# zzuiekongning/MGDT-YOLO

Measured on AMD Instinct MI355X. Metric: images/sec @640x640 bs=32 per GPU, detection forward + NMS (whole job: 1 GPU(s)), higher is better.
Workload: dtype bf16; 1 GPU; mspa_c2f_gd_yolov8-n (MSPA-C2f + GD neck + Detect, nc=80) 640x640 inference, batch 32/GPU: forward + decode + NMS(conf 0.25, iou 0.7), hipGraph replay, 4 batches in flight (one captured graph per resident batch, replayed round-robin on 4 streams); global_batch=32, parallelism=replicas x1 (batch-sharded, no data-path collective), rccl_ranks=1, input=bfloat16 NCHW images, 8 different batches resident in HBM (600 MiB) cycled, detections_last_step=9600, weights=seeded random init (no checkpoints offline), batches_in_flight=4

## Files before the change

### mgdt_yolo_amd/csrc/csp_block.hip

```cpp
#include <algorithm>
#include <vector>

#include "conv_igemm_kernel.h"

struct CspArgs {
  const char* x; int xsn, xsh, xsw; uint32_t x_bytes;
  char* y; int ysn, ysh, ysw; uint32_t y_bytes;
  const char* front; const float* front_bias;
  const char* mid[4]; const float* mid_bias[4];
  const char* back; const float* back_bias;
  float* pool;
  int N, H, W, Cin, Cout, wd, nbtl, shortcut, act;
  int TH, TW, halo, RH, RW, tiles_x, tiles_y, total_tiles, per_xcd;
  int catC, nchb, nbo;
  int RPA, TPA, CS;
  int catS, cmsk, csh;
  int chain_words;
  unsigned long long* dbg;
  int pool_gst;
  FastDiv fd_rw, fd_tw, fd_tx, fd_tpi;
};

constexpr int CSP_THREADS = 512;
constexpr int CSP_NW = CSP_THREADS / 64;
constexpr int CSP_NCHB_MAX = 8;

__device__ __forceinline__ float csp_act(float v, int) { return v * fast_sigmoid(v); }

typedef __attribute__((__vector_size__(2 * sizeof(unsigned int)))) unsigned int csp_raw2;

__device__ __forceinline__ void lds_store4(char* p, f32x4 v) {
  bf16x4 o;
#pragma unroll
  for (int i = 0; i < 4; ++i) o[i] = (bf16)v[i];
  *(bf16x4*)p = o;
}
template <int WD> __device__ __forceinline__ int csp_psw(int pix) { return WD == 64 ? (pix & 7) : (WD == 32 ? ((pix >> 1) & 3) : 0); }

__device__ __forceinline__ f32x4 lds_load4(const char* p) {
  const bf16x4 o = *(const bf16x4*)p;
  return f32x4{(float)o[0], (float)o[1], (float)o[2], (float)o[3]};
}

__device__ __forceinline__ csp_raw2 csp_swap32(unsigned int lo, unsigned int hi) { return __builtin_amdgcn_permlane32_swap(lo, hi, false, false); }
__device__ __forceinline__ f32x4 csp_merge(f32x4 va, f32x4 vb) {
  f32x4 m;
#pragma unroll
  for (int j = 0; j < 4; ++j) {
    const float fa = va[j], fb = vb[j];
    m[j] = __uint_as_float(csp_swap32(__float_as_uint(fa), __float_as_uint(fb))[0]);
  }
  return m;
}

template <int WD, int MODE, bool PAIR = false>
__global__ __launch_bounds__(CSP_THREADS, (WD <= 32 ? 4 : 2)) void csp_block_kernel(const CspArgs a) {
  static_assert(!PAIR || (WD == 8 && MODE == 0), "the paired epilogue is the wd = 8 MSPA form");
  constexpr int CP = WD / 8;
  constexpr int NCHB = WD == 8 ? 2 : (WD == 16 ? 3 : (WD == 32 ? 5 : 8));
  constexpr int NB = WD >= 16 ? WD / 16 : 1;
  constexpr int NCH = (9 * CP + 3) / 4;
  constexpr int NBK = NB, KC = (NBK + 1) / 2;
  constexpr int PS = 2 * WD;
  extern __shared__ __attribute__((aligned(16))) char smem[];
  char* Pb = smem;
  char* Tb = Pb + (size_t)a.RPA * PS;
  char* catb = Tb + (size_t)a.RPA * PS;
  char* wl = catb + (size_t)a.TPA * a.CS;

  const int tid = threadIdx.x, lane = tid & 63;
  const int wave = __builtin_amdgcn_readfirstlane(tid >> 6);
  const int r = lane & 15, g = lane >> 4;

  const int v = blockIdx.x;
  const int tlin = (v & 7) * a.per_xcd + (v >> 3);
  if ((v >> 3) >= a.per_xcd || tlin >= a.total_tiles) return;
  const int tpi = a.tiles_x * a.tiles_y;
  const int n = (int)fdiv((uint32_t)tlin, a.fd_tpi), trem = tlin - n * tpi;
  const int tyi = (int)fdiv((uint32_t)trem, a.fd_tx);
  const int ty0 = tyi * a.TH, tx0 = (trem - tyi * a.tiles_x) * a.TW;
  const int RP = a.RH * a.RW, TP = a.TH * a.TW;
  const bool inner = ty0 >= a.halo && tx0 >= a.halo && ty0 + a.TH + a.halo <= a.H && tx0 + a.TW + a.halo <= a.W;
  auto stamp = [&](int k) __attribute__((always_inline)) { if (a.dbg && tid == 0) a.dbg[(size_t)tlin * 8 + k] = __builtin_amdgcn_s_memrealtime(); };
  auto region_px = [&](int q, int& go, int& ct) __attribute__((always_inline)) {
    const int ry = (int)fdiv((uint32_t)q, a.fd_rw), rx = q - ry * a.RW;
    const int iy = ty0 - a.halo + ry, ix = tx0 - a.halo + rx;
    go = (q < RP && (unsigned)iy < (unsigned)a.H && (unsigned)ix < (unsigned)a.W) ? n * a.xsn + iy * a.xsh + ix * a.xsw : MGDT_OOB;
    const int cy = ry - a.halo, cx = rx - a.halo;
    ct = (q < RP && (unsigned)cy < (unsigned)a.TH && (unsigned)cx < (unsigned)a.TW) ? cy * a.TW + cx : -1;
  };
  auto pt_at = [&](int q, int c) __attribute__((always_inline)) { return q * PS + ((((c >> 3) ^ csp_psw<WD>(q)) << 4) | ((c & 7) << 1)); };
  auto cat_at = [&](int t, int c) __attribute__((always_inline)) { return t * a.CS + ((((c >> 3) ^ ((t >> a.csh) & a.cmsk)) << 4) | ((c & 7) << 1)); };
  stamp(0);

  const int nbv = wave % NB, gvm = wave / NB, gstm = CSP_NW / NB;
  bf16x8 A[NCH];
  f32x4 bias;
  auto load_a0 = [&]() __attribute__((always_inline)) {
#pragma unroll
    for (int kc = 0; kc < NCH; ++kc) A[kc] = *(const bf16x8*)(a.mid[0] + ((size_t)(kc * NB + nbv) * 64 + lane) * 16);
    bias = *(const f32x4*)(a.mid_bias[0] + nbv * 16 + 4 * g);
  };
  if (WD != 32 || MODE != 0) load_a0();

  {
    const int words = (int)(((size_t)2 * a.RPA * PS) >> 4);
    uint4* z = (uint4*)Pb;
    for (int i = tid; i < words; i += CSP_THREADS) z[i] = make_uint4(0u, 0u, 0u, 0u);
  }
  if (MODE == 0) {
    for (int i = tid; i < a.chain_words; i += CSP_THREADS) ((uint4*)wl)[i] = ((const uint4*)a.front)[i];
    float* bl = (float*)(wl + (size_t)a.chain_words * 16);
    for (int i = tid; i < 3 * NBK * 16; i += CSP_THREADS) bl[i] = ((const float*)(a.front + (size_t)a.chain_words * 16))[i];
  }
  __syncthreads();
  stamp(1);

  const __amdgpu_buffer_rsrc_t xrs = __builtin_amdgcn_make_buffer_rsrc((void*)a.x, 0, a.x_bytes, 0x00020000);
  const __amdgpu_buffer_rsrc_t yrs = __builtin_amdgcn_make_buffer_rsrc((void*)a.y, 0, a.y_bytes, 0x00020000);
  const int ngr = (RP + 15) >> 4;

  if (MODE == 0) {
    constexpr int U = WD == 64 ? 2 : (WD == 32 ? 3 : 5);
    const char* const wlane = wl + lane * 16;
    const float* bl = (const float*)(wl + (size_t)a.chain_words * 16);
    const int per = ngr / CSP_NW, rem = ngr - per * CSP_NW;
    const int gbeg = wave * per + min(wave, rem), gend = gbeg + per + (wave < rem ? 1 : 0);
    if constexpr (PAIR) {
      constexpr int UP = 3;
      const int hb = lane >> 5, cl = 4 * (g & 1);
      for (int g0 = gbeg; g0 < gend; g0 += 2 * UP) {
        int go[UP], ct[UP];
        csp_raw2 XR[UP][4];
#pragma unroll
        for (int u = 0; u < UP; ++u) {
          const int grp = g0 + 2 * u + hb;
          region_px(grp * 16 + r, go[u], ct[u]);
          if (grp >= gend) go[u] = MGDT_OOB, ct[u] = -1;
#pragma unroll
          for (int i = 0; i < 4; ++i) XR[u][i] = __builtin_amdgcn_raw_buffer_load_b64(xrs, (uint32_t)go[u] + (uint32_t)((i * WD + cl) * 2), 0, 0);
        }
#pragma unroll
        for (int u = 0; u < UP; ++u) {
          if (g0 + 2 * u >= gend) break;
          const bool hasb = g0 + 2 * u + 1 < gend;
          const int q = (g0 + 2 * u + hb) * 16 + r;
          f32x4 X[4];
#pragma unroll
          for (int i = 0; i < 4; ++i) {
            const bf16x4 o = __builtin_bit_cast(bf16x4, XR[u][i]);
            X[i] = f32x4{(float)o[0], (float)o[1], (float)o[2], (float)o[3]};
          }
          f32x4 prev;
#pragma unroll
          for (int i = 0; i < 3; ++i) {
            bf16x4 vb;
#pragma unroll
            for (int e = 0; e < 4; ++e) vb[e] = (bf16)(X[i][e] + (i ? prev[e] : 0.f));
            const csp_raw2 vw = __builtin_bit_cast(csp_raw2, vb);
            const csp_raw2 s0 = csp_swap32(vw[0], 0u), s1 = csp_swap32(vw[1], 0u);
            typedef __attribute__((__vector_size__(4 * sizeof(unsigned int)))) unsigned int raw4;
            const bf16x8 Ba = __builtin_bit_cast(bf16x8, (raw4){s0[0], s1[0], 0u, 0u});
            const bf16x8 Bb = __builtin_bit_cast(bf16x8, (raw4){s0[1], s1[1], 0u, 0u});
            const f32x4 bi = *(const f32x4*)(bl + i * 16 + 4 * g);
            const bf16x8 Wf = *(const bf16x8*)(wlane + i * 1024);
            const f32x4 acca = mma(Wf, Ba, bi);
            f32x4 accb = bi;
            if (hasb) accb = mma(Wf, Bb, bi);
            f32x4 acc = csp_merge(acca, accb);
#pragma unroll
            for (int j = 0; j < 4; ++j) acc[j] = (float)(bf16)csp_act(acc[j], a.act);
            prev = acc;
            if (ct[u] >= 0) lds_store4(catb + cat_at(ct[u], i * WD + cl), acc);
          }
          f32x4 p0 = prev + X[3];
          if (go[u] == MGDT_OOB) p0 = f32x4{0.f, 0.f, 0.f, 0.f};
          if (hb == 0 || hasb) lds_store4(Pb + pt_at(q, cl), p0);
        }
      }
    } else
    for (int g0 = gbeg; g0 < gend; g0 += U) {
      int go[U], ct[U];
      csp_raw2 XR[U][4][NBK];
#pragma unroll
      for (int u = 0; u < U; ++u) {
        const bool gv_ = g0 + u < gend;
        const int q = (g0 + u) * 16 + r;
        region_px(q, go[u], ct[u]);
        if (!gv_) go[u] = MGDT_OOB, ct[u] = -1;
#pragma unroll
        for (int i = 0; i < 4; ++i)
#pragma unroll
          for (int blk = 0; blk < NBK; ++blk) {
            const int c = blk * 16 + 4 * g;
            const int dead = c >= WD ? MGDT_OOB : 0;
            XR[u][i][blk] = __builtin_amdgcn_raw_buffer_load_b64(xrs, (uint32_t)(go[u] | dead) + (uint32_t)((i * WD + c) * 2), 0, 0);
          }
      }
#pragma unroll
      for (int u = 0; u < U; ++u) {
        if (g0 + u >= gend) break;
        const int q = (g0 + u) * 16 + r;
        f32x4 X[4][NBK];
#pragma unroll
        for (int i = 0; i < 4; ++i)
#pragma unroll
          for (int blk = 0; blk < NBK; ++blk) {
            const bf16x4 o = __builtin_bit_cast(bf16x4, XR[u][i][blk]);
            X[i][blk] = f32x4{(float)o[0], (float)o[1], (float)o[2], (float)o[3]};
          }
        f32x4 prev[NBK];
#pragma unroll
        for (int i = 0; i < 3; ++i) {
          bf16x8 Bf[KC];
#pragma unroll
          for (int kc = 0; kc < KC; ++kc)
#pragma unroll
            for (int e = 0; e < 8; ++e) {
              const int blk = kc * 2 + e / 4;
              float vv = 0.f;
              if (blk < NBK) vv = X[i][blk][e % 4] + (i ? prev[blk][e % 4] : 0.f);
              Bf[kc][e] = (bf16)vv;
            }
#pragma unroll
          for (int ob = 0; ob < NBK; ++ob) {
            f32x4 acc = *(const f32x4*)(bl + (i * NBK + ob) * 16 + 4 * g);
#pragma unroll
            for (int kc = 0; kc < KC; ++kc) acc = mma(*(const bf16x8*)(wlane + ((i * KC + kc) * NBK + ob) * 1024), Bf[kc], acc);
#pragma unroll
            for (int j = 0; j < 4; ++j) acc[j] = (float)(bf16)csp_act(acc[j], a.act);
            prev[ob] = acc;
            const int c = ob * 16 + 4 * g;
            if (c < WD && ct[u] >= 0) lds_store4(catb + cat_at(ct[u], i * WD + c), acc);
          }
        }
#pragma unroll
        for (int ob = 0; ob < NBK; ++ob) {
          const int c = ob * 16 + 4 * g;
          f32x4 p0 = prev[ob] + X[3][ob];
          if (go[u] == MGDT_OOB) p0 = f32x4{0.f, 0.f, 0.f, 0.f};
          if (c < WD) lds_store4(Pb + pt_at(q, c), p0);
        }
      }
    }
  } else {
    constexpr int NB2 = 2 * WD / 16;
    constexpr int U = WD == 64 ? 2 : 4;
    const int per = ngr / CSP_NW, rem = ngr - per * CSP_NW;
    const int gbeg = wave * per + min(wave, rem), gend = gbeg + per + (wave < rem ? 1 : 0);
    for (int g0 = gbeg; g0 < gend; g0 += U) {
      int go[U], ct[U];
      csp_raw2 XR[U][NB2];
#pragma unroll
      for (int u = 0; u < U; ++u) {
        const bool gv_ = g0 + u < gend;
        const int q = (g0 + u) * 16 + r;
        region_px(q, go[u], ct[u]);
        if (!gv_) go[u] = MGDT_OOB, ct[u] = -1;
#pragma unroll
        for (int blk = 0; blk < NB2; ++blk)
          XR[u][blk] = __builtin_amdgcn_raw_buffer_load_b64(xrs, (uint32_t)go[u] + (uint32_t)((blk * 16 + 4 * g) * 2), 0, 0);
      }
#pragma unroll
      for (int u = 0; u < U; ++u) {
        if (g0 + u >= gend) break;
        const int q = (g0 + u) * 16 + r;
#pragma unroll
        for (int blk = 0; blk < NB2; ++blk) {
          const int cc = blk * 16 + 4 * g;
          if (ct[u] >= 0) *(csp_raw2*)(catb + cat_at(ct[u], cc)) = XR[u][blk];
          if (cc >= WD) *(csp_raw2*)(Pb + pt_at(q, cc - WD)) = XR[u][blk];
        }
      }
    }
  }
  if (WD == 32 && MODE == 0) load_a0();
  stamp(2);
  __syncthreads();
  stamp(3);

  constexpr bool PREB = WD <= 16;
  bf16x8 AB[NCHB];
  f32x4 biasB = f32x4{0.f, 0.f, 0.f, 0.f};
  const int bgst = a.pool_gst, bgv = wave / (CSP_NW / bgst), obst = CSP_NW / bgst, ob0 = wave % obst;
  {
    const int gv = gvm, gst = gstm;
    const int cch = nbv * 16 + 4 * g;
    const int slot0 = (MODE == 0 ? 3 : 2) * WD;
    for (int j = 0; j < 2 * a.nbtl; ++j) {
      const char* in = (j & 1) ? Tb : Pb;
      char* out = (j & 1) ? Pb : Tb;
      constexpr bool PREN = WD <= 16;
      bf16x8 An[PREN ? NCH : 1];
      f32x4 biasn = bias;
      const bool more = j + 1 < 2 * a.nbtl;
      if (more) {
        if (PREN) {
#pragma unroll
          for (int kc = 0; kc < NCH; ++kc) An[kc] = *(const bf16x8*)(a.mid[j + 1] + ((size_t)(kc * NB + nbv) * 64 + lane) * 16);
          biasn = *(const f32x4*)(a.mid_bias[j + 1] + nbv * 16 + 4 * g);
        }
      } else if (PREB && ob0 < a.nbo) {
#pragma unroll
        for (int kc = 0; kc < NCHB; ++kc)
          if (kc < a.nchb) AB[kc] = *(const bf16x8*)(a.back + ((size_t)(kc * a.nbo + ob0) * 64 + lane) * 16);
        biasB = *(const f32x4*)(a.back_bias + ob0 * 16 + 4 * g);
      }
      const int lo = (j + 1) * a.RW + (j + 1), hi = (a.RH - j - 2) * a.RW + (a.RW - j - 1);
      const int ng = (hi - lo + 15) >> 4;
      const bool second = j & 1;
      const bool tocat = second && (j >> 1) + 1 < a.nbtl;
      const bool zchk = !inner && j + 1 < 2 * a.nbtl;
      int boff[NCH];
#pragma unroll
      for (int kc = 0; kc < NCH; ++kc) {
        const int p = kc * 4 + g;
        int tap = p / CP, cp = p - tap * CP;
        if (tap >= 9) { tap = 4; cp = 0; }
        const int toff = (tap / 3 - 1) * a.RW + (tap % 3 - 1);
        boff[kc] = toff * PS + ((cp ^ csp_psw<WD>(lo + r + toff)) << 4);
      }
      auto finish = [&](int q, f32x4 acc, int cc, bool live) __attribute__((always_inline)) {
#pragma unroll
        for (int jj = 0; jj < 4; ++jj) acc[jj] = csp_act(acc[jj], a.act);
        if (live && q < hi && cc < WD) {
          char* po = out + pt_at(q, cc);
          if (second && a.shortcut) acc += lds_load4(po);
          int go = 0, ct = -1;
          if (zchk || tocat) region_px(q, go, ct);
          if (zchk && go == MGDT_OOB) acc = f32x4{0.f, 0.f, 0.f, 0.f};
          lds_store4(po, acc);
          if (tocat && ct >= 0) lds_store4(catb + cat_at(ct, slot0 + (j >> 1) * WD + cc), acc);
        }
      };
      for (int grp = gv; grp < ng; grp += 2 * gst) {
        const int qa = lo + grp * 16 + r;
        const bool hasb = grp + gst < ng;
        const int qb = hasb ? qa + gst * 16 : qa;
        const char* pa = in + qa * PS;
        const char* pb = in + qb * PS;
        f32x4 acca = bias, accb = bias;
#pragma unroll
        for (int kc = 0; kc < NCH; ++kc) {
          acca = mma(A[kc], *(const bf16x8*)(pa + boff[kc]), acca);
          accb = mma(A[kc], *(const bf16x8*)(pb + boff[kc]), accb);
        }
        if constexpr (PAIR) {
          finish(lane < 32 ? qa : qb, csp_merge(acca, accb), 4 * (g & 1), lane < 32 || hasb);
        } else {
          finish(qa, acca, cch, true);
          if (hasb) finish(qb, accb, cch, true);
        }
      }
      __syncthreads();
      if (j == 0) stamp(4);
      if (more) {
        if (PREN) {
#pragma unroll
          for (int kc = 0; kc < NCH; ++kc) A[kc] = An[kc];
          bias = biasn;
        } else {
#pragma unroll
          for (int kc = 0; kc < NCH; ++kc) A[kc] = *(const bf16x8*)(a.mid[j + 1] + ((size_t)(kc * NB + nbv) * 64 + lane) * 16);
          bias = *(const f32x4*)(a.mid_bias[j + 1] + nbv * 16 + 4 * g);
        }
      }
    }
  }
  stamp(5);

  {
    const int tg = (TP + 15) >> 4;
    const int nsl = a.catS >> 3, csw = (r >> a.csh) & a.cmsk;
    int koff[NCHB];
    bool kinp[NCHB];
#pragma unroll
    for (int kc = 0; kc < NCHB; ++kc) {
      const int p = kc * 4 + g;
      kinp[kc] = p >= nsl && p < nsl + CP;
      koff[kc] = kinp[kc] ? p - nsl : ((p < nsl ? p : 0) ^ csw) << 4;
    }
    const int gst = bgst, gv = bgv;
    bf16x8 ABn[PREB ? 1 : NCHB];
    f32x4 biasBn = biasB;
    if (!PREB && ob0 < a.nbo) {
#pragma unroll
      for (int kc = 0; kc < NCHB; ++kc)
        if (kc < a.nchb) AB[kc] = *(const bf16x8*)(a.back + ((size_t)(kc * a.nbo + ob0) * 64 + lane) * 16);
      biasB = *(const f32x4*)(a.back_bias + ob0 * 16 + 4 * g);
    }
    for (int ob = ob0; ob < a.nbo; ob += obst) {
      if (PREB && ob != ob0) {
#pragma unroll
        for (int kc = 0; kc < NCHB; ++kc)
          if (kc < a.nchb) AB[kc] = *(const bf16x8*)(a.back + ((size_t)(kc * a.nbo + ob) * 64 + lane) * 16);
        biasB = *(const f32x4*)(a.back_bias + ob * 16 + 4 * g);
      }
      if (!PREB && ob + obst < a.nbo) {
#pragma unroll
        for (int kc = 0; kc < NCHB; ++kc)
          if (kc < a.nchb) ABn[kc] = *(const bf16x8*)(a.back + ((size_t)(kc * a.nbo + ob + obst) * 64 + lane) * 16);
        biasBn = *(const f32x4*)(a.back_bias + (ob + obst) * 16 + 4 * g);
      }
      const int co = ob * 16 + 4 * g;
      const int dead = co >= a.Cout ? MGDT_OOB : 0;
      f32x4 psum = f32x4{0.f, 0.f, 0.f, 0.f};
      for (int grp = gv; grp < tg; grp += gst) {
        const int t = grp * 16 + r;
        const int tc = min(t, TP - 1);
        const int cy = (int)fdiv((uint32_t)tc, a.fd_tw), cx = tc - cy * a.TW;
        const int tq = (cy + a.halo) * a.RW + cx + a.halo;
        const int yo = t < TP ? n * a.ysn + (ty0 + cy) * a.ysh + (tx0 + cx) * a.ysw : MGDT_OOB;
        const char* pc = catb + t * a.CS;
        const char* pp = Pb + tq * PS;
        const int psw = csp_psw<WD>(tq);
        f32x4 acc = biasB;
#pragma unroll
        for (int kc = 0; kc < NCHB; ++kc)
          if (kc < a.nchb) acc = mma(AB[kc], *(const bf16x8*)(kinp[kc] ? pp + ((koff[kc] ^ psw) << 4) : pc + koff[kc]), acc);
#pragma unroll
        for (int jj = 0; jj < 4; ++jj) acc[jj] = (float)(bf16)csp_act(acc[jj], a.act);
        bstore4<bf16>(yrs, (uint32_t)(yo | dead) + (uint32_t)(co * 2), acc);
        if (t < TP) psum += acc;
      }
      if (a.pool) {
#pragma unroll
        for (int m = 1; m < 16; m <<= 1)
#pragma unroll
          for (int jj = 0; jj < 4; ++jj) psum[jj] += __shfl_xor(psum[jj], m, 64);
        if (r == 0 && co < a.Cout) {
          *(f32x4*)(a.pool + (((size_t)n * tpi + trem) * gst + gv) * a.Cout + co) = psum;
        }
      }
      if (!PREB && ob + obst < a.nbo) {
#pragma unroll
        for (int kc = 0; kc < NCHB; ++kc) AB[kc] = ABn[kc];
        biasB = biasBn;
      }
    }
  }
  stamp(6);
}

struct CspGeom { int TH, TW, halo, RH, RW, RPA, TPA, CS, tiles_x, tiles_y; size_t lds; };

static void csp_cat_swizzle(int slots, int* cmsk, int* csh) {
  if (slots % 16 == 0) { *cmsk = 15; *csh = 0; }
  else if (slots % 8 == 0) { *cmsk = 7; *csh = 0; }
  else if (slots % 4 == 0) { *cmsk = 3; *csh = 1; }
  else { *cmsk = 0; *csh = 0; }
}

static bool csp_geometry(int mode, int H, int W, int wd, int nbtl, int catC, size_t extra, int th, int tw, CspGeom* g) {
  g->TH = th; g->TW = tw; g->halo = 2 * nbtl;
  g->RH = th + 2 * g->halo; g->RW = tw + 2 * g->halo;
  const int RP = g->RH * g->RW;
  g->RPA = ((RP + 15 + 15) / 16) * 16;
  g->TPA = ((th * tw + 15) / 16) * 16;
  g->CS = (catC - wd) * 2;
  g->tiles_x = W / tw; g->tiles_y = H / th;
  g->lds = 2 * (size_t)g->RPA * (wd * 2) + (size_t)g->TPA * g->CS + extra;
  (void)mode;
  return g->lds <= 156 * 1024;
}

static int csp_chain_nbk(int wd) { return wd >= 16 ? wd / 16 : 1; }
static int csp_pool_gst(int cout) { const int nbo = (cout + 15) / 16; return (nbo < CSP_NW && CSP_NW % nbo == 0) ? CSP_NW / nbo : 1; }

int csp_c3_supported(int cin, int cout, int wd, int nbtl, int h, int w, int dtype);
int csp_c3_tiles(int n, int cin, int cout, int wd, int nbtl, int h, int w, int* geom8);
int csp_c3_fwd(const mgdt_view* x, const void* const* mid, const float* const* mid_bias, int nbtl, int shortcut, const void* back, const float* back_bias,
               int wd, const mgdt_view* y, mgdt_stream s);

extern "C" int mgdt_csp_block_supported(int mode, int cin, int cout, int wd, int nbtl, int h, int w, int dtype) {
  if (mode == 2) return csp_c3_supported(cin, cout, wd, nbtl, h, w, dtype);
  if (mode != 0 && mode != 1) return 0;
  if (dtype != MGDT_BF16 || (wd != 8 && wd != 16 && wd != 32 && wd != 64) || nbtl < 1 || nbtl > 2 || cout % 4) return 0;
  const int catC = (mode == 0 ? 3 : 2) * wd + nbtl * wd;
  if (catC > 256 || catC % 8) return 0;
  if (mode == 0) {
    if (cin != 4 * wd || h % 2 || w % 2 || h < 4 || w < 4) return 0;
  } else {
    if (cin != 2 * wd || wd < 16) return 0;
  }
  return 1;
}

constexpr size_t CSP_LDS_2WG = 80 * 1024;
constexpr double CSP_1WG_COST = 2.0;

static bool csp_pick_tile(int mode, int H, int W, int N, int wd, int nbtl, int catC, size_t extra, CspGeom* best) {
  const char* e = getenv("MGDT_CSP_TILE");
  int fth = 0, ftw = 0;
  if (e && sscanf(e, "%d,%d", &fth, &ftw) != 2) fth = ftw = 0;
  const int qh = mode == 0 ? H / 2 : H, qw = mode == 0 ? W / 2 : W;
  double best_cost = 1e30;
  bool found = false;
  for (int th = 2; th <= std::min(qh, 32); ++th) {
    if (qh % th) continue;
    for (int tw = 2; tw <= std::min(qw, 32); ++tw) {
      if (qw % tw) continue;
      if (fth && (th != fth || tw != ftw)) continue;
      CspGeom g;
      if (!csp_geometry(mode, H, W, wd, nbtl, catC, extra, th, tw, &g)) continue;
      const double wgs = (double)N * g.tiles_x * g.tiles_y;
      const double ratio = (double)(g.RH * g.RW) / (th * tw);
      const double fill = (double)(th * tw) / g.TPA;
      double cost = ratio / fill;
      if (wgs < 256) cost *= 256.0 / wgs;
      if (wd <= 32 && g.lds > CSP_LDS_2WG) cost *= CSP_1WG_COST;
      if (cost < best_cost) { best_cost = cost; *best = g; found = true; }
    }
  }
  return found;
}

extern "C" int mgdt_csp_block_tiles(int mode, int n, int cin, int cout, int wd, int nbtl, int h, int w, int* geom6) {
  if (mode == 2) return csp_c3_tiles(n, cin, cout, wd, nbtl, h, w, geom6);
  if (!mgdt_csp_block_supported(mode, cin, cout, wd, nbtl, h, w, MGDT_BF16)) return 0;
  const int catC = (mode == 0 ? 3 : 2) * wd + nbtl * wd;
  const int nbk = csp_chain_nbk(wd);
  const size_t extra = mode == 0 ? (size_t)3 * ((nbk + 1) / 2) * nbk * 1024 + 3 * nbk * 16 * 4 : 0;
  CspGeom g;
  if (!csp_pick_tile(mode, h, w, n, wd, nbtl, catC, extra, &g)) return 0;
  if (geom6) {
    geom6[0] = g.TH; geom6[1] = g.TW; geom6[2] = g.RH; geom6[3] = g.RW; geom6[4] = (int)g.lds; geom6[5] = n * g.tiles_x * g.tiles_y;
    geom6[6] = g.tiles_x; geom6[7] = g.tiles_y;
  }
  return g.tiles_x * g.tiles_y * csp_pool_gst(cout);
}

extern "C" int mgdt_csp_block_fwd(int mode, const mgdt_view* x, const void* front, const float* front_bias, const void* const* mid,
                                  const float* const* mid_bias, int nbtl, int shortcut, const void* back, const float* back_bias, int wd, int act,
                                  const mgdt_view* y, float* pool, int dtype, mgdt_stream s) {
  if (!view_ok(x) || !view_ok(y) || (mode == 0 && !front) || !mid || !mid_bias || !back || !back_bias) MGDT_FAIL(MGDT_BAD_ARG, "csp_block: null/empty argument");
  if (!mgdt_csp_block_supported(mode, x->c, y->c, wd, nbtl, x->h, x->w, dtype))
    MGDT_FAIL(MGDT_BAD_SHAPE, "csp_block: mode=%d cin=%d cout=%d wd=%d n=%d %dx%d dtype=%d not covered", mode, x->c, y->c, wd, nbtl, x->h, x->w, dtype);
  if (x->n != y->n || x->h != y->h || x->w != y->w) MGDT_FAIL(MGDT_BAD_SHAPE, "csp_block: x and y must have one spatial size");
  if (act != MGDT_ACT_SILU) MGDT_FAIL(MGDT_BAD_ARG, "csp_block: activation %d (only SiLU, the blocks' default, is built)", act);
  for (int j = 0; j < 2 * nbtl; ++j)
    if (!mid[j] || !mid_bias[j]) MGDT_FAIL(MGDT_BAD_ARG, "csp_block: missing conv panel %d", j);
  if (mode == 2) return csp_c3_fwd(x, mid, mid_bias, nbtl, shortcut, back, back_bias, wd, y, s);
  CspArgs a;
  memset(&a, 0, sizeof(a));
  const long sz = 2;
  bool fits = true;
  auto bind = [&](const mgdt_view* v, const char** p, int* sn, int* sh, int* sw, uint32_t* bytes, int q) {
    const long ext = ((long)(v->n - 1) * v->sn + (long)(v->h - 1) * v->sh + (long)(v->w - 1) * v->sw + v->c) * sz;
    if (v->sc != 1 || v->sw % q || v->sh % q || v->sn % q || (uintptr_t)v->p % (q * sz) || ext >= 0x7fffffffL) { fits = false; return; }
    *p = (const char*)v->p; *sn = (int)(v->sn * sz); *sh = (int)(v->sh * sz); *sw = (int)(v->sw * sz); *bytes = (uint32_t)ext;
  };
  const char* yp = nullptr;
  bind(x, &a.x, &a.xsn, &a.xsh, &a.xsw, &a.x_bytes, 4);
  bind(y, &yp, &a.ysn, &a.ysh, &a.ysw, &a.y_bytes, 4);
  if (!fits) MGDT_FAIL(MGDT_BAD_SHAPE, "csp_block: views must be aligned NHWC (sc == 1) and span < 2 GiB");
  a.y = (char*)yp;
  a.front = (const char*)front; a.front_bias = front_bias;
  for (int j = 0; j < 2 * nbtl; ++j) { a.mid[j] = (const char*)mid[j]; a.mid_bias[j] = mid_bias[j]; }
  a.back = (const char*)back; a.back_bias = back_bias; a.pool = pool;
  a.N = x->n; a.H = x->h; a.W = x->w; a.Cin = x->c; a.Cout = y->c; a.wd = wd; a.nbtl = nbtl; a.shortcut = shortcut; a.act = act;
  a.catC = (mode == 0 ? 3 : 2) * wd + nbtl * wd;
  a.nchb = (a.catC / 8 + 3) / 4; a.nbo = (a.Cout + 15) / 16; a.pool_gst = csp_pool_gst(a.Cout);
  const int nbk = csp_chain_nbk(wd);
  a.chain_words = mode == 0 ? 3 * ((nbk + 1) / 2) * nbk * 64 : 0;
  const size_t extra = mode == 0 ? (size_t)a.chain_words * 16 + 3 * nbk * 16 * 4 : 0;
  CspGeom g;
  if (!csp_pick_tile(mode, a.H, a.W, a.N, wd, nbtl, a.catC, extra, &g)) MGDT_FAIL(MGDT_BAD_SHAPE, "csp_block: no tile fits %dx%d wd=%d n=%d", a.H, a.W, wd, nbtl);
  a.TH = g.TH; a.TW = g.TW; a.halo = g.halo; a.RH = g.RH; a.RW = g.RW; a.tiles_x = g.tiles_x; a.tiles_y = g.tiles_y;
  a.RPA = g.RPA; a.TPA = g.TPA; a.CS = g.CS;
  a.catS = a.catC - wd;
  csp_cat_swizzle(a.catS / 8, &a.cmsk, &a.csh);
  a.total_tiles = a.N * g.tiles_x * g.tiles_y;
  a.fd_rw = make_fastdiv((uint32_t)g.RW); a.fd_tw = make_fastdiv((uint32_t)g.TW); a.fd_tx = make_fastdiv((uint32_t)g.tiles_x);
  a.fd_tpi = make_fastdiv((uint32_t)(g.tiles_x * g.tiles_y));
  a.per_xcd = cdiv(a.total_tiles, 8);
  const int grid = 8 * a.per_xcd;
  hipStream_t st = (hipStream_t)s;
  static unsigned long long* dbgbuf = nullptr;
  static size_t dbgcap = 0;
  if (getenv("MGDT_CSP_DBG") && dbgcap < (size_t)a.total_tiles * 8) {
    if (dbgbuf) (void)hipFree(dbgbuf);
    dbgcap = (size_t)a.total_tiles * 8;
    (void)hipMalloc((void**)&dbgbuf, dbgcap * 8);
  }
  a.dbg = getenv("MGDT_CSP_DBG") ? dbgbuf : nullptr;
  const char* ep = getenv("MGDT_CSP_PAIR");
  const bool pair = !(ep && ep[0] == '0');
#define CSP_LAUNCH(...)                                                                                              \
  do {                                                                                                                      \
    static std::atomic<bool> attr{false};                                                                                            \
    if (!attr) {                                                                                                            \
      hipError_t e_ = hipFuncSetAttribute((const void*)csp_block_kernel<__VA_ARGS__>, hipFuncAttributeMaxDynamicSharedMemorySize, 160 * 1024); \
      if (e_ != hipSuccess) MGDT_FAIL(MGDT_LAUNCH_FAIL, "csp_block: hipFuncSetAttribute: %s", hipGetErrorString(e_));         \
      attr = true;                                                                                                          \
    }                                                                                                                       \
    csp_block_kernel<__VA_ARGS__><<<grid, CSP_THREADS, g.lds, st>>>(a);                                                      \
  } while (0)
  if (mode == 0) {
    switch (wd) { case 8: if (pair) CSP_LAUNCH(8, 0, true); else CSP_LAUNCH(8, 0); break; case 16: CSP_LAUNCH(16, 0); break; case 32: CSP_LAUNCH(32, 0); break; default: CSP_LAUNCH(64, 0); break; }
  } else {
    switch (wd) { case 16: CSP_LAUNCH(16, 1); break; case 32: CSP_LAUNCH(32, 1); break; default: CSP_LAUNCH(64, 1); break; }
  }
#undef CSP_LAUNCH
  MGDT_CHECK_LAUNCH("csp_block_fwd");
  if (a.dbg) {
    std::vector<unsigned long long> h((size_t)a.total_tiles * 8);
    (void)hipStreamSynchronize(st);
    (void)hipMemcpy(h.data(), a.dbg, h.size() * 8, hipMemcpyDeviceToHost);
    unsigned long long t0 = ~0ull, t1 = 0;
    double ph[6] = {0, 0, 0, 0, 0, 0};
    for (int i = 0; i < a.total_tiles; ++i) {
      t0 = std::min(t0, h[(size_t)i * 8]); t1 = std::max(t1, h[(size_t)i * 8 + 6]);
      for (int k = 0; k < 6; ++k) ph[k] += (double)(h[(size_t)i * 8 + k + 1] - h[(size_t)i * 8 + k]);
    }
    const double nw = a.total_tiles;
    fprintf(stderr, "csp_block mode %d wd %d n %d %dx%d tile %dx%d (%d wgs, lds %zu): span %.1f us; avg per WG (us): tables %.2f front %.2f sync %.2f conv0 %.2f "
                    "other convs %.2f back %.2f\n", mode, wd, nbtl, a.H, a.W, g.TH, g.TW, a.total_tiles, g.lds, (t1 - t0) * 0.01, ph[0] / nw * 0.01,
            ph[1] / nw * 0.01, ph[2] / nw * 0.01, ph[3] / nw * 0.01, ph[4] / nw * 0.01, ph[5] / nw * 0.01);
  }
  return MGDT_OK;
}
```

Before: 40380 images/sec.

## Compact halo-shrinking conv walk and re-swizzle LDS reads in fused CSP block

The chained 3x3 convs in the fused CSP block now iterate only over the valid shrinking interior pixels. A fast division by the per-stage width maps a compact index back to region coordinates, so work is no longer wasted on row-wrap pixels between lo and hi. For wd>=32 the LDS read offsets use an XOR swizzle computed per pixel address, and weight and bias prefetch for the next stage or the back conv is moved before the barrier. The loop is split at compile time so the last stage is specialised, and occupancy for the paired wd=8 form rises to 6 waves per SIMD. The cost is extra integer work per pixel group and higher register pressure.

```diff
diff --git a/mgdt_yolo_amd/csrc/csp_block.hip b/mgdt_yolo_amd/csrc/csp_block.hip
--- a/mgdt_yolo_amd/csrc/csp_block.hip
+++ b/mgdt_yolo_amd/csrc/csp_block.hip
@@ -1,4 +1,5 @@
 #include <algorithm>
+#include <type_traits>
 #include <vector>
 
 #include "conv_igemm_kernel.h"
@@ -19,11 +20,13 @@
   unsigned long long* dbg;
   int pool_gst;
   FastDiv fd_rw, fd_tw, fd_tx, fd_tpi;
+  FastDiv fd_cw[4];
 };
 
 constexpr int CSP_THREADS = 512;
 constexpr int CSP_NW = CSP_THREADS / 64;
 constexpr int CSP_NCHB_MAX = 8;
+constexpr int csp_waves_per_simd(int wd, bool pair) { return wd == 8 && pair ? 6 : (wd <= 32 ? 4 : 2); }
 
 __device__ __forceinline__ float csp_act(float v, int) { return v * fast_sigmoid(v); }
 
@@ -53,8 +56,8 @@
   return m;
 }
 
-template <int WD, int MODE, bool PAIR = false>
-__global__ __launch_bounds__(CSP_THREADS, (WD <= 32 ? 4 : 2)) void csp_block_kernel(const CspArgs a) {
+template <int WD, int MODE, bool PAIR = false, bool COMPACT = true>
+__global__ __launch_bounds__(CSP_THREADS, csp_waves_per_simd(WD, PAIR)) void csp_block_kernel(const CspArgs a) {
   static_assert(!PAIR || (WD == 8 && MODE == 0), "the paired epilogue is the wd = 8 MSPA form");
   constexpr int CP = WD / 8;
   constexpr int NCHB = WD == 8 ? 2 : (WD == 16 ? 3 : (WD == 32 ? 5 : 8));
@@ -280,6 +283,11 @@
   stamp(3);
 
   constexpr bool PREB = WD <= 16;
+  constexpr int NPRE = WD <= 16 ? NCH : 0;
+  constexpr int NPREB = PREB ? NCHB : 0;
+  constexpr bool RESW = COMPACT && WD >= 32;
+  constexpr int CPL = CP >= 4 ? CP / 4 : 1;
+  constexpr int SWM = WD == 64 ? 0x70 : 0x30;
   bf16x8 AB[NCHB];
   f32x4 biasB = f32x4{0.f, 0.f, 0.f, 0.f};
   const int bgst = a.pool_gst, bgv = wave / (CSP_NW / bgst), obst = CSP_NW / bgst, ob0 = wave % obst;
@@ -287,30 +295,38 @@
     const int gv = gvm, gst = gstm;
     const int cch = nbv * 16 + 4 * g;
     const int slot0 = (MODE == 0 ? 3 : 2) * WD;
-    for (int j = 0; j < 2 * a.nbtl; ++j) {
+    auto conv3 = [&](const int j, auto LAST) __attribute__((always_inline)) {
       const char* in = (j & 1) ? Tb : Pb;
       char* out = (j & 1) ? Pb : Tb;
-      constexpr bool PREN = WD <= 16;
-      bf16x8 An[PREN ? NCH : 1];
+      bf16x8 An[NPRE > 0 ? NPRE : 1];
       f32x4 biasn = bias;
-      const bool more = j + 1 < 2 * a.nbtl;
-      if (more) {
-        if (PREN) {
-#pragma unroll
-          for (int kc = 0; kc < NCH; ++kc) An[kc] = *(const bf16x8*)(a.mid[j + 1] + ((size_t)(kc * NB + nbv) * 64 + lane) * 16);
-          biasn = *(const f32x4*)(a.mid_bias[j + 1] + nbv * 16 + 4 * g);
-        }
-      } else if (PREB && ob0 < a.nbo) {
-#pragma unroll
-        for (int kc = 0; kc < NCHB; ++kc)
+      constexpr bool more = !decltype(LAST)::value;
+      if constexpr (more) {
+#pragma unroll
+        for (int kc = 0; kc < NPRE; ++kc) An[kc] = *(const bf16x8*)(a.mid[j + 1] + ((size_t)(kc * NB + nbv) * 64 + lane) * 16);
+        biasn = *(const f32x4*)(a.mid_bias[j + 1] + nbv * 16 + 4 * g);
+      } else if (ob0 < a.nbo) {
+#pragma unroll
+        for (int kc = 0; kc < NPREB; ++kc)
           if (kc < a.nchb) AB[kc] = *(const bf16x8*)(a.back + ((size_t)(kc * a.nbo + ob0) * 64 + lane) * 16);
         biasB = *(const f32x4*)(a.back_bias + ob0 * 16 + 4 * g);
       }
       const int lo = (j + 1) * a.RW + (j + 1), hi = (a.RH - j - 2) * a.RW + (a.RW - j - 1);
-      const int ng = (hi - lo + 15) >> 4;
+      const int wj = a.RW - 2 * j - 2, npx = (a.RH - 2 * j - 2) * wj;
+      const int ng = COMPACT ? (npx + 15) >> 4 : (hi - lo + 15) >> 4;
+      const FastDiv fdw = a.fd_cw[j];
+      auto gpx = [&](int grp, bool& lv) __attribute__((always_inline)) {
+        const int idx = grp * 16 + r;
+        lv = true;
+        if constexpr (!COMPACT) return lo + idx;
+        lv = idx < npx;
+        const int ic = min(idx, npx - 1);
+        const int row = (int)fdiv((uint32_t)ic, fdw);
+        return lo + row * a.RW + (ic - row * wj);
+      };
       const bool second = j & 1;
       const bool tocat = second && (j >> 1) + 1 < a.nbtl;
-      const bool zchk = !inner && j + 1 < 2 * a.nbtl;
+      const bool zchk = !inner && more;
       int boff[NCH];
 #pragma unroll
       for (int kc = 0; kc < NCH; ++kc) {
@@ -318,8 +334,12 @@
         int tap = p / CP, cp = p - tap * CP;
         if (tap >= 9) { tap = 4; cp = 0; }
         const int toff = (tap / 3 - 1) * a.RW + (tap % 3 - 1);
-        boff[kc] = toff * PS + ((cp ^ csp_psw<WD>(lo + r + toff)) << 4);
-      }
+        boff[kc] = toff * PS + ((RESW ? cp : cp ^ csp_psw<WD>(lo + r + toff)) << 4);
+      }
+      auto bsw = [&](int q, int tap) __attribute__((always_inline)) {
+        const int X = q * PS + boff[tap * CPL];
+        return X ^ ((X >> 3) & SWM);
+      };
       auto finish = [&](int q, f32x4 acc, int cc, bool live) __attribute__((always_inline)) {
 #pragma unroll
         for (int jj = 0; jj < 4; ++jj) acc[jj] = csp_act(acc[jj], a.act);
@@ -334,38 +354,53 @@
         }
       };
       for (int grp = gv; grp < ng; grp += 2 * gst) {
-        const int qa = lo + grp * 16 + r;
         const bool hasb = grp + gst < ng;
-        const int qb = hasb ? qa + gst * 16 : qa;
-        const char* pa = in + qa * PS;
-        const char* pb = in + qb * PS;
+        bool lva, lvb;
+        const int qa = gpx(grp, lva);
+        const int qb = gpx(hasb ? grp + gst : grp, lvb);
         f32x4 acca = bias, accb = bias;
-#pragma unroll
-        for (int kc = 0; kc < NCH; ++kc) {
-          acca = mma(A[kc], *(const bf16x8*)(pa + boff[kc]), acca);
-          accb = mma(A[kc], *(const bf16x8*)(pb + boff[kc]), accb);
+        if constexpr (RESW) {
+#pragma unroll
+          for (int tap = 0; tap < 9; ++tap) {
+            const int oa = bsw(qa, tap), ob = bsw(qb, tap);
+#pragma unroll
+            for (int h = 0; h < CPL; ++h) {
+              acca = mma(A[tap * CPL + h], *(const bf16x8*)(in + (oa ^ (h << 6))), acca);
+              accb = mma(A[tap * CPL + h], *(const bf16x8*)(in + (ob ^ (h << 6))), accb);
+            }
+          }
+        } else {
+          const char* pa = in + qa * PS;
+          const char* pb = in + qb * PS;
+#pragma unroll
+          for (int kc = 0; kc < NCH; ++kc) {
+            acca = mma(A[kc], *(const bf16x8*)(pa + boff[kc]), acca);
+            accb = mma(A[kc], *(const bf16x8*)(pb + boff[kc]), accb);
+          }
         }
         if constexpr (PAIR) {
-          finish(lane < 32 ? qa : qb, csp_merge(acca, accb), 4 * (g & 1), lane < 32 || hasb);
+          finish(lane < 32 ? qa : qb, csp_merge(acca, accb), 4 * (g & 1), lane < 32 ? lva : hasb && lvb);
         } else {
-          finish(qa, acca, cch, true);
-          if (hasb) finish(qb, accb, cch, true);
-        }
+          finish(qa, acca, cch, lva);
+          if (hasb) finish(qb, accb, cch, lvb);
+        }
+      }
+      if constexpr (more) {
+#pragma unroll
+        for (int kc = 0; kc < NPRE; ++kc) A[kc] = An[kc];
+#pragma unroll
+        for (int kc = NPRE; kc < NCH; ++kc) A[kc] = *(const bf16x8*)(a.mid[j + 1] + ((size_t)(kc * NB + nbv) * 64 + lane) * 16);
+        bias = biasn;
+      } else if (ob0 < a.nbo) {
+#pragma unroll
+        for (int kc = NPREB; kc < NCHB; ++kc)
+          if (kc < a.nchb) AB[kc] = *(const bf16x8*)(a.back + ((size_t)(kc * a.nbo + ob0) * 64 + lane) * 16);
       }
       __syncthreads();
       if (j == 0) stamp(4);
-      if (more) {
-        if (PREN) {
-#pragma unroll
-          for (int kc = 0; kc < NCH; ++kc) A[kc] = An[kc];
-          bias = biasn;
-        } else {
-#pragma unroll
-          for (int kc = 0; kc < NCH; ++kc) A[kc] = *(const bf16x8*)(a.mid[j + 1] + ((size_t)(kc * NB + nbv) * 64 + lane) * 16);
-          bias = *(const f32x4*)(a.mid_bias[j + 1] + nbv * 16 + 4 * g);
-        }
-      }
-    }
+    };
+    for (int j = 0; j + 1 < 2 * a.nbtl; ++j) conv3(j, std::false_type{});
+    conv3(2 * a.nbtl - 1, std::true_type{});
   }
   stamp(5);
 
@@ -383,12 +418,6 @@
     const int gst = bgst, gv = bgv;
     bf16x8 ABn[PREB ? 1 : NCHB];
     f32x4 biasBn = biasB;
-    if (!PREB && ob0 < a.nbo) {
-#pragma unroll
-      for (int kc = 0; kc < NCHB; ++kc)
-        if (kc < a.nchb) AB[kc] = *(const bf16x8*)(a.back + ((size_t)(kc * a.nbo + ob0) * 64 + lane) * 16);
-      biasB = *(const f32x4*)(a.back_bias + ob0 * 16 + 4 * g);
-    }
     for (int ob = ob0; ob < a.nbo; ob += obst) {
       if (PREB && ob != ob0) {
 #pragma unroll
@@ -573,6 +602,7 @@
   a.total_tiles = a.N * g.tiles_x * g.tiles_y;
   a.fd_rw = make_fastdiv((uint32_t)g.RW); a.fd_tw = make_fastdiv((uint32_t)g.TW); a.fd_tx = make_fastdiv((uint32_t)g.tiles_x);
   a.fd_tpi = make_fastdiv((uint32_t)(g.tiles_x * g.tiles_y));
+  for (int j = 0; j < 2 * nbtl; ++j) a.fd_cw[j] = make_fastdiv((uint32_t)(g.RW - 2 * j - 2));
   a.per_xcd = cdiv(a.total_tiles, 8);
   const int grid = 8 * a.per_xcd;
   hipStream_t st = (hipStream_t)s;
@@ -586,6 +616,8 @@
   a.dbg = getenv("MGDT_CSP_DBG") ? dbgbuf : nullptr;
   const char* ep = getenv("MGDT_CSP_PAIR");
   const bool pair = !(ep && ep[0] == '0');
+  const char* ec = getenv("MGDT_CSP_COMPACT");
+  const bool compact = !(ec && ec[0] == '0');
 #define CSP_LAUNCH(...)                                                                                              \
   do {                                                                                                                      \
     static std::atomic<bool> attr{false};                                                                                            \
@@ -596,11 +628,13 @@
     }                                                                                                                       \
     csp_block_kernel<__VA_ARGS__><<<grid, CSP_THREADS, g.lds, st>>>(a);                                                      \
   } while (0)
+#define CSP_WALK(...) do { if (compact) CSP_LAUNCH(__VA_ARGS__, true); else CSP_LAUNCH(__VA_ARGS__, false); } while (0)
   if (mode == 0) {
-    switch (wd) { case 8: if (pair) CSP_LAUNCH(8, 0, true); else CSP_LAUNCH(8, 0); break; case 16: CSP_LAUNCH(16, 0); break; case 32: CSP_LAUNCH(32, 0); break; default: CSP_LAUNCH(64, 0); break; }
+    switch (wd) { case 8: if (pair) CSP_WALK(8, 0, true); else CSP_WALK(8, 0, false); break; case 16: CSP_WALK(16, 0, false); break; case 32: CSP_WALK(32, 0, false); break; default: CSP_WALK(64, 0, false); break; }
   } else {
-    switch (wd) { case 16: CSP_LAUNCH(16, 1); break; case 32: CSP_LAUNCH(32, 1); break; default: CSP_LAUNCH(64, 1); break; }
-  }
+    switch (wd) { case 16: CSP_WALK(16, 1, false); break; case 32: CSP_WALK(32, 1, false); break; default: CSP_WALK(64, 1, false); break; }
+  }
+#undef CSP_WALK
 #undef CSP_LAUNCH
   MGDT_CHECK_LAUNCH("csp_block_fwd");
   if (a.dbg) {
```

Result: faster. 41820 images/sec, median of 6 (+3.6%).
